# hashicorp/consul

Measured on NVIDIA H100. Metric: million node-ticks/sec, higher is better.
Workload: dtype u32

## Files before the change

### consul_b200/csrc/gs_cuda.cu

```cuda
#include <cuda_runtime.h>
#include <stdio.h>
#include <stdlib.h>
#include <string.h>

#include <map>

#include "gs_aux.h"
#include "gs_backend.h"
#include "gs_query.h"
#include "gs_vmm.h"

#define GS_BLOCK 256
#define GS_GRAPH_TICKS 64
#define GS_WIN_GRAPH 8
#ifndef GS_STRETCH_TICKS
#define GS_STRETCH_TICKS 16
#endif

namespace {

template <bool COORDS>
struct DevSinkT {
  static constexpr bool kCoords = COORDS;
  uint32_t* s_stat;
  uint32_t* s_heard;
  uint32_t* s_q;
  __device__ __forceinline__ void activity() { s_q[0] = 1u; }
  __device__ __forceinline__ void horizon(uint32_t h) { atomicMin(&s_q[1], h); }
  __device__ __forceinline__ void stat(int idx, uint32_t v) { atomicAdd(&s_stat[idx * 32 + (threadIdx.x & 31u)], v); }
  __device__ __forceinline__ void heard(uint32_t r) { atomicAdd(&s_heard[r * 32u + (threadIdx.x & 31u)], 1u); }
  __device__ __forceinline__ void crashed_dead(const GsDev& d, uint32_t t) {
    uint32_t old = atomicSub_system(d.crashed_alive, 1u);
    if (old == 1u) *d.crashed_dead_tick = t;
  }
  __device__ __forceinline__ void log_event(const GsDev& d, const GsGlobals& g, uint32_t t,
                                            uint32_t type, uint32_t subject, uint32_t observer,
                                            uint32_t ltime) {
    uint32_t pos = atomicAdd_system(&d.evlog_cursor[0], 1u);
    if (pos < g.evlog_cap) {
      GsEventRec e;
      e.tick = t;
      e.type = type;
      e.subject = subject;
      e.observer = observer;
      e.ltime = ltime;
      e.reserved = 0u;
      d.evlog[pos] = e;
    } else {
      atomicAdd_system(&d.evlog_cursor[1], 1u);
    }
  }
};
typedef DevSinkT<false> DevSink;

#ifndef GS_MIN_BLOCKS
#define GS_MIN_BLOCKS 4
#endif
#define GS_WARPS (GS_BLOCK / 32)
#define GS_ROUND 4

__device__ __forceinline__ uint32_t gs_smem_addr(const void* p) { return (uint32_t)__cvta_generic_to_shared(p); }
__device__ __forceinline__ void gs_mbar_init(uint64_t* bar, uint32_t arrivals) {
  asm volatile("mbarrier.init.shared::cta.b64 [%0], %1;" ::"r"(gs_smem_addr(bar)), "r"(arrivals) : "memory");
}
__device__ __forceinline__ void gs_mbar_expect_tx(uint64_t* bar, uint32_t bytes) {
  asm volatile("mbarrier.arrive.expect_tx.shared::cta.b64 _, [%0], %1;" ::"r"(gs_smem_addr(bar)), "r"(bytes) : "memory");
}
__device__ __forceinline__ void gs_bulk_g2s(void* smem_dst, const void* gsrc, uint32_t bytes, uint64_t* bar) {
  asm volatile("cp.async.bulk.shared::cluster.global.mbarrier::complete_tx::bytes [%0], [%1], %2, [%3];" ::"r"(
                   gs_smem_addr(smem_dst)),
               "l"(gsrc), "r"(bytes), "r"(gs_smem_addr(bar))
               : "memory");
}
__device__ __forceinline__ bool gs_mbar_wait(uint64_t* bar, uint32_t parity) {
  for (uint32_t spin = 0; spin < (1u << 24); ++spin) {
    uint32_t done;
    asm volatile(
        "{\n\t.reg .pred p;\n\t"
        "mbarrier.try_wait.parity.shared::cta.b64 p, [%1], %2;\n\t"
        "selp.u32 %0, 1, 0, p;\n\t}"
        : "=r"(done)
        : "r"(gs_smem_addr(bar)), "r"(parity)
        : "memory");
    if (done) return true;
  }
  return false;
}

__device__ __forceinline__ void gs_ranks_wait(const GsDev& d, const GsGlobals& g, uint32_t t) {
  if (threadIdx.x < g.world) {
    uint32_t v;
    do {
      asm volatile("ld.acquire.sys.global.u32 %0, [%1];" : "=r"(v) : "l"(d.tick_flags[g.rank] + threadIdx.x) : "memory");
    } while ((int32_t)(v - t) < 0);
  }
  __syncthreads();
}
__device__ __forceinline__ void gs_ranks_release(const GsDev& d, const GsGlobals& g, uint32_t t_done) {
  __syncthreads();
  if (threadIdx.x == 0u) {
    __threadfence_system();
    const uint32_t arrived = atomicAdd(d.done_ctr, 1u);
    if (arrived == gridDim.x - 1u) {
      __threadfence_system();
      *d.done_ctr = 0u;
      __threadfence_system();
      for (uint32_t r = 0; r < g.world; ++r)
        asm volatile("st.release.sys.global.u32 [%0], %1;" ::"l"(d.tick_flags[r] + g.rank), "r"(t_done) : "memory");
    }
  }
}

__device__ __forceinline__ void gs_q_publish(const GsDev& d, const GsGlobals& g, const uint32_t* s_q, uint32_t t) {
  if (s_q[0] != 0u) {
    if (g.world <= 1u) atomicMax(d.qstate[0] + GS_Q_LAST_ACTIVE, t + 1u);
    else for (uint32_t r = 0; r < g.world; ++r) atomicMax_system(d.qstate[r] + GS_Q_LAST_ACTIVE, t + 1u);
  }
  if (s_q[1] != GS_NEVER) {
    if (g.world <= 1u) atomicMin(d.qstate[0] + GS_Q_HORIZON, s_q[1]);
    else for (uint32_t r = 0; r < g.world; ++r) atomicMin_system(d.qstate[r] + GS_Q_HORIZON, s_q[1]);
  }
}

template <bool COORDS>
__device__ __noinline__ void gs_row_step_impaired_call(const GsDev* dp, const GsGlobals* gp, uint32_t i, uint32_t t,
                                                       uint32_t inb, uint32_t* s_stat, uint32_t* s_heard, uint32_t* s_q) {
  DevSinkT<COORDS> sink{s_stat, s_heard, s_q};
  gs_row_step_body<true>(*dp, *gp, i, t, t % gp->GI, inb, sink);
}
template <bool COORDS>
__device__ __noinline__ void gs_row_step_call(const GsDev* dp, const GsGlobals* gp, uint32_t i, uint32_t t,
                                              uint32_t inb, uint32_t* s_stat, uint32_t* s_heard, uint32_t* s_q) {
  if (dp->imp_loss != nullptr) {
    gs_row_step_impaired_call<COORDS>(dp, gp, i, t, inb, s_stat, s_heard, s_q);
    return;
  }
  DevSinkT<COORDS> sink{s_stat, s_heard, s_q};
  gs_row_step_body<false>(*dp, *gp, i, t, t % gp->GI, inb, sink);
}

struct GsStretchCtl {
  GsStretch out;
  uint32_t violation;
  uint32_t end, floor, depth;
};
__device__ __forceinline__ uint32_t gs_stretch_stop(const GsStretchCtl& c, uint32_t last_active) {
  const uint32_t quiet_at = (last_active > c.floor ? last_active : c.floor) + c.depth;
  return quiet_at < c.end ? quiet_at : c.end;
}

template <bool COORDS>
__global__ void __launch_bounds__(GS_BLOCK, GS_MIN_BLOCKS)
    gs_tick_kernel(const __grid_constant__ GsDev d, const GsGlobals* __restrict__ gp, uint32_t k_off,
                   const GsStretchCtl* __restrict__ stretch) {
  __shared__ uint32_t s_stat[GS_NSTAT * 32];
  __shared__ uint32_t s_heard[32 * 32];
  __shared__ __align__(128) uint32_t s_inb[GS_WARPS][GS_ROUND][GS_TILE];
  __shared__ __align__(128) uint32_t s_due[GS_WARPS][GS_ROUND][GS_TILE];
  __shared__ __align__(8) uint64_t s_bar[GS_WARPS];
  __shared__ uint32_t s_q[2];
  __shared__ uint32_t s_work[GS_WARPS * GS_ROUND * 4];
  __shared__ uint32_t s_wn[2], s_wtake[2];
  const uint32_t tid = threadIdx.x;
  for (uint32_t x = tid; x < GS_NSTAT * 32u; x += GS_BLOCK) s_stat[x] = 0u;
  for (uint32_t x = tid; x < 32u * 32u; x += GS_BLOCK) s_heard[x] = 0u;
  if (tid == 64u) s_q[0] = 0u;
  if (tid == 65u) s_q[1] = GS_NEVER;
  if (tid >= 66u && tid < 68u) s_wn[tid - 66u] = 0u;
  if (tid >= 68u && tid < 70u) s_wtake[tid - 68u] = 0u;
  if (tid >= 96u && tid < 96u + GS_WARPS) gs_mbar_init(&s_bar[tid - 96u], 1u);
  asm volatile("fence.mbarrier_init.release.cluster;" ::: "memory");
  asm volatile("griddepcontrol.launch_dependents;" ::: "memory");
  asm volatile("griddepcontrol.wait;" ::: "memory");
  if (stretch != nullptr && *d.tick_base + k_off >= gs_stretch_stop(*stretch, __ldcg(d.qstate[0] + GS_Q_LAST_ACTIVE)))
    return;
  __syncthreads();
  const GsGlobals& g = *gp;
  const uint32_t t = *d.tick_base + k_off;
  if (g.world > 1u) gs_ranks_wait(d, g, t);
  const uint32_t cur = t & 1u, P = g.P, pslot = t % P, gslot = t % g.GI;
  const uint32_t pslot_t = (t + P - g.T % P) % P;
  const uint32_t lane = tid & 31u, wib = tid >> 5;
  uint32_t tile_lo = 0, tile_hi = (g.n + GS_TILE - 1u) / GS_TILE;
  if (g.world > 1u) {
    const uint32_t per = g.rows_per_rank / GS_TILE;
    tile_lo = g.rank * per < tile_hi ? g.rank * per : tile_hi;
    tile_hi = tile_lo + per < tile_hi ? tile_lo + per : tile_hi;
  }
  const uint32_t n_warps = gridDim.x * GS_WARPS, n_tiles = tile_hi - tile_lo;
  const uint32_t wid = blockIdx.x * GS_WARPS + wib;
  const uint32_t t_begin = tile_lo + (uint32_t)(((uint64_t)wid * n_tiles) / n_warps);
  const uint32_t t_end = tile_lo + (uint32_t)(((uint64_t)(wid + 1u) * n_tiles) / n_warps);
  const uint32_t* __restrict__ inbox_cur = d.inbox[t & g.ring_mask];
  const bool gated = g.phase_gate != 0u;
  const uint32_t shift = g.phase_shift;
  DevSinkT<COORDS> sink{s_stat, s_heard, s_q};

  const uint32_t max_run = (n_tiles + n_warps - 1u) / n_warps, n_rounds = (max_run + GS_ROUND - 1u) / GS_ROUND;
  bool did_work = false;
  const bool sys_scan = g.world > 1u && (g.flags & 4u);
  auto bring = [&](uint32_t r) {
    const uint32_t b0 = t_begin + r * GS_ROUND < t_end ? t_begin + r * GS_ROUND : t_end;
    const uint32_t b1 = b0 + GS_ROUND < t_end ? b0 + GS_ROUND : t_end;
    const uint32_t tiles = b1 - b0;
    if (!tiles) return;
    uint32_t gate_mask = 0;
    for (uint32_t x = 0; x < tiles; ++x) {
      bool gate = true;
      if (gated) {
        const uint32_t pp = gs_probe_phase(g.rot_p, (b0 + x) >> shift, P);
        gate = pp == pslot || pp == pslot_t;
      }
      gate_mask |= gate ? 1u << x : 0u;
    }
    const size_t off0 = (size_t)b0 * GS_TILE;
    if (sys_scan) {
      for (uint32_t x = 0; x < tiles; ++x) {
        uint4 v;
        asm volatile("ld.relaxed.sys.global.v4.u32 {%0,%1,%2,%3}, [%4];"
                     : "=r"(v.x), "=r"(v.y), "=r"(v.z), "=r"(v.w) : "l"(inbox_cur + off0 + x * GS_TILE + lane * 4u) : "memory");
        *reinterpret_cast<uint4*>(&s_inb[wib][x][lane * 4u]) = v;
        const uint4 dv = (gate_mask >> x) & 1u ? *reinterpret_cast<const uint4*>(d.due + off0 + x * GS_TILE + lane * 4u)
                                               : make_uint4(GS_NEVER, GS_NEVER, GS_NEVER, GS_NEVER);
        *reinterpret_cast<uint4*>(&s_due[wib][x][lane * 4u]) = dv;
      }
      __syncwarp();
      return;
    }
    for (uint32_t x = 0; x < tiles; ++x)
      if (!((gate_mask >> x) & 1u))
        *reinterpret_cast<uint4*>(&s_due[wib][x][lane * 4u]) = make_uint4(GS_NEVER, GS_NEVER, GS_NEVER, GS_NEVER);
    __syncwarp();
    if (lane == 0u) {
      asm volatile("fence.proxy.async.shared::cta;" ::: "memory");
      gs_mbar_expect_tx(&s_bar[wib], (tiles + __popc(gate_mask)) * GS_TILE * 4u);
      gs_bulk_g2s(&s_inb[wib][0][0], inbox_cur + off0, tiles * GS_TILE * 4u, &s_bar[wib]);
      for (uint32_t x = 0; x < tiles; ++x)
        if ((gate_mask >> x) & 1u) gs_bulk_g2s(&s_due[wib][x][0], d.due + off0 + x * GS_TILE, GS_TILE * 4u, &s_bar[wib]);
    }
  };
  bring(0u);
  for (uint32_t round = 0; round < n_rounds; ++round) {
  const uint32_t par = round & 1u;
  const uint32_t r_begin = t_begin + round * GS_ROUND < t_end ? t_begin + round * GS_ROUND : t_end;
  const uint32_t r_end = r_begin + GS_ROUND < t_end ? r_begin + GS_ROUND : t_end;
  if (r_end > r_begin && !sys_scan && !gs_mbar_wait(&s_bar[wib], round & 1u)) {
    if (lane == 0u) atomicExch(d.qstate[g.rank] + GS_Q_VIOLATION, t + 1u);
  }
  for (uint32_t tile = r_begin; tile < r_end; ++tile) {
    const uint32_t st = tile - r_begin;
    uint4 i4 = *reinterpret_cast<const uint4*>(&s_inb[wib][st][lane * 4u]);
    const uint4 d4 = *reinterpret_cast<const uint4*>(&s_due[wib][st][lane * 4u]);
    if (__any_sync(0xFFFFFFFFu, (i4.x | i4.y | i4.z | i4.w) != 0u)) {
      const uint32_t m0 = tile * GS_TILE + lane * 4u;
      const uint4 h4 = __ldcg(reinterpret_cast<const uint4*>(d.heard + m0));
      uint32_t* const w_cur = d.inbox[t & g.ring_mask] + m0;
      uint32_t* const w4 = &i4.x;
      const uint32_t* const h = &h4.x;
      const uint32_t* const du = &d4.x;
      bool stale_any = false;
#pragma unroll
      for (uint32_t u = 0; u < 4u; ++u) {
        const bool pp = g.pp_interval != 0u && gs_pp_due(g.pp_interval, g.rot_pp, (m0 + u) / g.phase_group, t);
        if (w4[u] != 0u && gs_mail_is_stale(g, w4[u], h[u], du[u] == t, pp)) {
          w_cur[u] = 0u;
          s_inb[wib][st][lane * 4u + u] = 0u;
          w4[u] = 0u;
          stale_any = true;
        }
      }
      if (stale_any) sink.activity();
    }
    bool mine = (i4.x | i4.y | i4.z | i4.w) != 0u || d4.x == t || d4.y == t || d4.z == t || d4.w == t;
    bool pp_tile = false;
    if (g.pp_interval != 0u) {
      if (gated) {
        pp_tile = gs_pp_due(g.pp_interval, g.rot_pp, tile >> shift, t);
      } else {
#pragma unroll
        for (uint32_t u = 0; u < 4u; ++u)
          pp_tile |= gs_pp_due(g.pp_interval, g.rot_pp, (tile * GS_TILE + lane * 4u + u) / g.phase_group, t);
      }
      mine |= pp_tile;
    }
    if (__any_sync(0xFFFFFFFFu, mine)) {
      did_work = true;
      __syncwarp();
      const uint32_t base = tile * GS_TILE + lane;
      bool act[4], cand[4];
      bool any_cand = false;
#pragma unroll
      for (int u = 0; u < 4; ++u) {
        const uint32_t w = s_inb[wib][st][u * 32 + lane];
        const bool due_now = s_due[wib][st][u * 32 + lane] == t;
        act[u] = w != 0u || due_now ||
                 (g.pp_interval != 0u && gs_pp_due(g.pp_interval, g.rot_pp, (base + 32u * u) / g.phase_group, t));
        cand[u] = w == 0u && due_now;
        any_cand |= cand[u];
      }
      if (__any_sync(0xFFFFFFFFu, any_cand)) {
        GsFastProbe f[4];
#pragma unroll
        for (int u = 0; u < 4; ++u)
          if (cand[u]) gs_fast_load(d, cur, base + 32u * u, f[u]);
#pragma unroll
        for (int u = 0; u < 4; ++u)
          if (cand[u]) cand[u] = gs_fast_target(d, g, cur, base + 32u * u, f[u]);
        uint32_t n_probe = 0, n_ack = 0;
#pragma unroll
        for (int u = 0; u < 4; ++u) {
          bool acked = false;
          const bool done = cand[u] && gs_fast_finish(d, g, sink, base + 32u * u, t, f[u], &acked);
          if (done) act[u] = false;
          n_probe += __popc(__ballot_sync(0xFFFFFFFFu, done));
          n_ack += __popc(__ballot_sync(0xFFFFFFFFu, done && acked));
        }
        if (lane == 0u && n_probe) {
          atomicAdd(&s_stat[GS_ST_PROBES * 32], n_probe);
          atomicAdd(&s_stat[GS_ST_ACTIVE_ROWS * 32], n_probe);
          if (n_ack) atomicAdd(&s_stat[GS_ST_ACKS * 32], n_ack);
        }
      }
#pragma unroll
      for (int u = 0; u < 4; ++u) {
        if (__any_sync(0xFFFFFFFFu, act[u]) && lane == 0u) s_work[atomicAdd(&s_wn[par], 1u)] = tile * 4u + (uint32_t)u;
      }
    }
  }
  __syncwarp();
  if (round + 1u < n_rounds) bring(round + 1u);
  __syncthreads();
  if (tid == 0u) s_wn[par ^ 1u] = s_wtake[par ^ 1u] = 0u;
  const uint32_t n_work = s_wn[par];
  for (;;) {
    uint32_t idx = 0;
    if (lane == 0u) idx = atomicAdd(&s_wtake[par], 1u);
    idx = __shfl_sync(0xFFFFFFFFu, idx, 0);
    if (idx >= n_work) break;
    did_work = true;
    const uint32_t i = s_work[idx] * 32u + lane;
    const uint32_t w = __ldcg(inbox_cur + i);
    const bool a = w != 0u || __ldcg(d.due + i) == t ||
                   (g.pp_interval != 0u && gs_pp_due(g.pp_interval, g.rot_pp, i / g.phase_group, t));
    if (a) gs_row_step_call<COORDS>(&d, gp, i, t, w, s_stat, s_heard, s_q);
  }
  __syncthreads();
  }
  if (g.world > 1u && did_work && !(g.flags & 8u)) __threadfence_system();
  __syncthreads();
  if (tid < GS_NSTAT) {
    uint32_t v = 0;
    for (uint32_t x = 0; x < 32u; ++x) v += s_stat[tid * 32u + ((x + tid) & 31u)];
    if (v) atomicAdd(&d.stats[tid], (unsigned long long)v);
  } else if (tid >= 32u && tid < 32u + GS_MAX_RUMORS) {
    uint32_t r = tid - 32u, c = 0;
    for (uint32_t x = 0; x < 32u; ++x) c += s_heard[r * 32u + ((x + r) & 31u)];
    if (c) {
      uint32_t old = atomicAdd_system(&d.heard_cnt[r], c);
      if (old + c == g.up_count) d.conv_tick[r] = t;
    }
  }
  if (tid == 0u) gs_q_publish(d, g, s_q, t);
  if (g.world > 1u) gs_ranks_release(d, g, t + 1u);
}

template <bool COORDS>
__device__ __noinline__ void gs_window_generic(const GsDev* dp, const GsGlobals* gp, uint32_t gb, uint32_t g_end,
                                               uint32_t tf00, uint32_t tf01, uint32_t tf02, uint32_t tf03,
                                               uint32_t tx00, uint32_t tx01, uint32_t tx02, uint32_t tx03,
                                               uint32_t t0, uint32_t w1, uint32_t* s_stat, uint32_t* s_heard,
                                               uint32_t* s_q, uint32_t* counts) {
  const GsDev& d = *dp;
  const GsGlobals& g = *gp;
  const GsHot h = gs_hot(g);
  const uint32_t P = h.P, T = h.T, lane = threadIdx.x & 31u;
  const uint32_t tf0[4] = {tf00, tf01, tf02, tf03}, tx0[4] = {tx00, tx01, tx02, tx03};
  const bool fast_ok =
      h.loss_thr == 0u && h.graph_n == 0u && d.coord == nullptr && d.imp_loss == nullptr && h.pp_interval == 0u;
  DevSinkT<COORDS> sink{s_stat, s_heard, s_q};
  uint32_t n_probe = 0, n_ack = 0;
  bool did_work = false;
  (void)did_work;
#pragma unroll 1
    for (uint32_t s0 = t0; s0 < w1; s0 += P) {
    const uint32_t off = s0 - t0;
    uint32_t tf[4], tx[4], due[4];
    bool cand[4], slow[4];
    bool any_slow = false;
#pragma unroll
    for (int u = 0; u < 4; ++u) {
      if (gb + u < g_end) {
        tf[u] = tf0[u] + off;
        tx[u] = tx0[u] + off;
        due[u] = __ldcg(d.due + (gb + u) * 32u + lane);
      } else {
        tf[u] = tx[u] = GS_NEVER;
        due[u] = GS_NEVER - 1u;
      }
      cand[u] = fast_ok && due[u] == tf[u] && tf[u] < w1;
      slow[u] = (due[u] == tf[u] && tf[u] < w1 && !fast_ok) || (due[u] == tx[u] && tx[u] < w1);
    }
    GsFastProbe f[4];
#pragma unroll
    for (int u = 0; u < 4; ++u)
      if (cand[u]) gs_fast_load(d, tf[u] & 1u, (gb + u) * 32u + lane, f[u]);
#pragma unroll
    for (int u = 0; u < 4; ++u)
      if (cand[u]) {
        const bool okk = gs_fast_target(d, h, tf[u] & 1u, (gb + u) * 32u + lane, f[u]);
        if (!okk) { cand[u] = false; slow[u] = true; }
      }
#pragma unroll
    for (int u = 0; u < 4; ++u) {
      bool acked = false, done = false;
      if (cand[u]) {
        done = gs_fast_finish(d, h, sink, (gb + u) * 32u + lane, tf[u], f[u], &acked);
        if (!done) slow[u] = true;
        else if (!acked && tf[u] + T < w1) slow[u] = true;
      }
      n_probe += done ? 1u : 0u;
      n_ack += done && acked ? 1u : 0u;
      any_slow |= slow[u];
    }
    if (__any_sync(0xFFFFFFFFu, any_slow)) {
      did_work = true;
#pragma unroll 1
      for (int u = 0; u < 4; ++u) {
        const bool sl = u == 0 ? slow[0] : u == 1 ? slow[1] : u == 2 ? slow[2] : slow[3];
        if (!__any_sync(0xFFFFFFFFu, sl)) continue;
        const uint32_t a = u == 0 ? tf[0] : u == 1 ? tf[1] : u == 2 ? tf[2] : tf[3];
        const uint32_t b = u == 0 ? tx[0] : u == 1 ? tx[1] : u == 2 ? tx[2] : tx[3];
        const uint32_t i = (gb + u) * 32u + lane;
#pragma unroll 1
        for (int which = 0; which < 2; ++which) {
          const uint32_t t = which == 0 ? (a < b ? a : b) : (a < b ? b : a);
          if (t >= w1) break;
          if (sl && __ldcg(d.due + i) == t) gs_row_step_call<COORDS>(&d, gp, i, t, 0u, s_stat, s_heard, s_q);
        }
      }
    }
    }
  counts[0] = n_probe;
  counts[1] = n_ack;
}

#ifndef GS_WIN_BLOCKS
#define GS_WIN_BLOCKS 4
#endif
#ifndef GS_WIN_BLOCKS_CLOSED
#define GS_WIN_BLOCKS_CLOSED 4
#endif

template <bool COORDS, bool PRISTINE>
__global__ void __launch_bounds__(GS_BLOCK, PRISTINE ? GS_WIN_BLOCKS_CLOSED : GS_WIN_BLOCKS)
    gs_window_kernel(const __grid_constant__ GsDev d, const GsGlobals* __restrict__ gp, uint32_t k_off, uint32_t n_ticks,
                     uint32_t mode) {
  __shared__ uint32_t s_stat[GS_NSTAT * 32];
  __shared__ uint32_t s_heard[32 * 32];
  __shared__ uint32_t s_q[2];
  __shared__ uint32_t s_spec[GS_MAX_SPECIAL + 1];
  const uint32_t tid = threadIdx.x;
  for (uint32_t x = tid; x < GS_NSTAT * 32u; x += GS_BLOCK) s_stat[x] = 0u;
  for (uint32_t x = tid; x < 32u * 32u; x += GS_BLOCK) s_heard[x] = 0u;
  if (tid == 64u) s_q[0] = 0u;
  if (tid == 65u) s_q[1] = GS_NEVER;
  asm volatile("griddepcontrol.launch_dependents;" ::: "memory");
  asm volatile("griddepcontrol.wait;" ::: "memory");
  if (tid == 66u) s_spec[GS_MAX_SPECIAL] = gs_special_members(*gp, s_spec);
  __syncthreads();
  const GsGlobals& g = *gp;
  const GsHot h = gs_hot(g);
  const bool cyclic = (mode & 2u) != 0u;
  const uint32_t world = g.world, rank = g.rank, n_spec = s_spec[GS_MAX_SPECIAL];
  uint32_t* const qs = d.qstate[rank];
  const uint32_t t0 = *d.tick_base + k_off;
  const uint32_t reached = __ldcg(qs + GS_Q_WIN_END), horizon = __ldcg(qs + GS_Q_HORIZON);
  if (reached < t0) return;
  uint32_t w1 = t0 + n_ticks;
  if (horizon < w1) w1 = horizon;
  if (w1 <= t0) return;
  if (world > 1u) gs_ranks_wait(d, g, t0);
  const uint32_t P = h.P, T = h.T, lane = tid & 31u, wib = tid >> 5;
  uint32_t tile_lo = 0, tile_hi = (h.n + GS_TILE - 1u) / GS_TILE;
  if (world > 1u) {
    const uint32_t per = g.rows_per_rank / GS_TILE;
    tile_lo = rank * per < tile_hi ? rank * per : tile_hi;
    tile_hi = tile_lo + per < tile_hi ? tile_lo + per : tile_hi;
  }
  const uint32_t n_warps = gridDim.x * GS_WARPS, grp_lo = tile_lo * 4u, grp_hi = tile_hi * 4u;
  const uint32_t run = (grp_hi - grp_lo + n_warps - 1u) / n_warps;
  const uint32_t wid = blockIdx.x * GS_WARPS + wib;
  const uint32_t g_begin = grp_lo + wid * run < grp_hi ? grp_lo + wid * run : grp_hi;
  const uint32_t g_end = g_begin + run < grp_hi ? g_begin + run : grp_hi;
  const uint32_t shift = g.phase_shift + 2u, t0_mod = t0 % P, rot_p = g.rot_p;
  const uint32_t win_q = (w1 - t0) / P, win_r = (w1 - t0) - win_q * P;
  const bool fast_ok =
      h.loss_thr == 0u && h.graph_n == 0u && d.coord == nullptr && d.imp_loss == nullptr && h.pp_interval == 0u;
  DevSinkT<COORDS> sink{s_stat, s_heard, s_q};
  bool did_work = false;
  uint32_t n_probe = 0, n_ack = 0;
  uint32_t pg = g_begin >> shift;
  uint32_t pp = (pg % P + rot_p) % P;
  const uint32_t g_first = cyclic ? (grp_lo + wid * 4u < grp_hi ? grp_lo + wid * 4u : grp_hi) : g_begin;
  const uint32_t g_step = cyclic ? n_warps * 4u : 4u, g_lim = cyclic ? grp_hi : g_end;
  for (uint32_t gb = g_first; gb < g_lim; gb += g_step) {
    if (cyclic) {
      pg = gb >> shift;
      pp = (pg % P + rot_p) % P;
    }
    uint32_t tf0[4], tx0[4];
#pragma unroll
    for (int u = 0; u < 4; ++u) {
      const uint32_t grp = gb + u;
      if (grp < g_lim) {
        const uint32_t q = grp >> shift;
        if (q != pg) {
          pp = pp + 1u == P ? 0u : pp + 1u;
          pg = q;
        }
        uint32_t a = pp + P - t0_mod;
        a = a >= P ? a - P : a;
        uint32_t b = a + T;
        b = b >= P ? b - P : b;
        tf0[u] = t0 + a;
        tx0[u] = t0 + b;
      } else {
        tf0[u] = tx0[u] = GS_NEVER;
      }
    }
    uint32_t lo = t0;
#pragma unroll 1
    for (;;) {
      uint32_t stuck = GS_NEVER;
      if constexpr (PRISTINE) {
        uint32_t cnt = 0;
        uint32_t du[4], kk[4], mm[4], cu[4], pa[4];
#pragma unroll
        for (int u = 0; u < 4; ++u) {
          const uint32_t i = (gb + u) * 32u + lane;
          du[u] = GS_NEVER;
          kk[u] = mm[u] = cu[u] = pa[u] = 0u;
          if (gb + u < g_lim) {
            du[u] = __ldcg(d.due + i);
            if (fast_ok) {
              kk[u] = d.key[tf0[u] & 1u][i];
              mm[u] = d.meta[i];
              cu[u] = d.cursor[i];
              pa[u] = d.pass[i];
            }
          }
        }
#pragma unroll
        for (int u = 0; u < 4; ++u) {
          if (gb + u >= g_lim) continue;
          const uint32_t i = (gb + u) * 32u + lane;
          uint32_t due = du[u];
          if (fast_ok && due >= lo && due < w1) {
            uint32_t later = 0u;
            bool on_phase = due == tf0[u];
            if (!on_phase && due > tf0[u]) {
              later = (due - tf0[u]) / P;
              on_phase = later * P == due - tf0[u];
            }
            if (on_phase) {
              const uint32_t k0 = ((due ^ tf0[u]) & 1u) ? d.key[due & 1u][i] : kk[u];
              const uint32_t m = mm[u];
              if (gs_key_truth(k0) == GS_TRUTH_UP && gs_key_rank(k0) == GS_RANK_ALIVE && gs_meta_stage(m) == GS_STAGE_IDLE &&
                  !(m & (GS_META_DIRTY | GS_META_ISOLATED))) {
                const GsU4 rk = gs_perm_keys(h.seed_lo, h.seed_hi, i, pa[u]);
                const uint32_t kt = win_q + (win_r > tf0[u] - t0 ? 1u : 0u) - later;
                const uint32_t k = gs_pristine_probes_k(h.n, h.perm_bits, rk, i, cu[u], kt, s_spec, n_spec);
                if (k) {
                  const uint32_t aw = gs_meta_aw(m);
                  if (aw) d.meta[i] = gs_meta_set_aw(m, aw > k ? aw - k : 0u);
                  d.cursor[i] = cu[u] + k;
                  due += k * P;
                  d.due[i] = due;
                  cnt += k;
                }
              }
            }
          }
          if (due >= lo && due < w1 && due < stuck) stuck = due;
        }
        n_probe += cnt;
        n_ack += cnt;
      } else
      {
        uint32_t mm[4], cu[4], du[4], m_in[4], cu_in[4], du_in[4], kt[4];
        GsU4 rk[4];
        bool live[4], in_rng[4];
        uint32_t cnt = 0;
        {
          uint32_t kk[4], pa[4];
#pragma unroll
          for (int u = 0; u < 4; ++u) {
            const uint32_t i = (gb + u) * 32u + lane;
            in_rng[u] = gb + u < g_lim;
            du[u] = GS_NEVER;
            kk[u] = mm[u] = cu[u] = pa[u] = 0u;
            if (in_rng[u]) {
              du[u] = __ldcg(d.due + i);
              if (fast_ok) {
                kk[u] = d.key[tf0[u] & 1u][i];
                mm[u] = d.meta[i];
                cu[u] = d.cursor[i];
                pa[u] = d.pass[i];
              }
            }
          }
#pragma unroll
          for (int u = 0; u < 4; ++u) {
            const uint32_t i = (gb + u) * 32u + lane;
            live[u] = false;
            kt[u] = 0u;
            m_in[u] = mm[u];
            cu_in[u] = cu[u];
            du_in[u] = du[u];
            if (!in_rng[u] || !fast_ok || du[u] < lo || du[u] >= w1) continue;
            uint32_t later = 0u;
            if (du[u] != tf0[u]) {
              if (du[u] < tf0[u]) continue;
              later = (du[u] - tf0[u]) / P;
              if (later * P != du[u] - tf0[u]) continue;
            }
            const uint32_t k = ((du[u] ^ tf0[u]) & 1u) ? d.key[du[u] & 1u][i] : kk[u];
            live[u] = gs_key_truth(k) == GS_TRUTH_UP && gs_key_rank(k) == GS_RANK_ALIVE &&
                      gs_meta_stage(mm[u]) == GS_STAGE_IDLE && !(mm[u] & (GS_META_DIRTY | GS_META_ISOLATED));
            rk[u] = gs_perm_keys(h.seed_lo, h.seed_hi, i, pa[u]);
            kt[u] = win_q + (win_r > tf0[u] - t0 ? 1u : 0u) - later;
          }
        }
        for (;;) {
          bool go[4];
          bool any = false;
#pragma unroll
          for (int u = 0; u < 4; ++u) {
            go[u] = live[u] && du[u] < w1;
            any |= go[u];
          }
          if (!__any_sync(0xFFFFFFFFu, any)) break;
          uint32_t c[4], kc[4];
#pragma unroll
          for (int u = 0; u < 4; ++u) {
            c[u] = 0u;
            if (go[u]) {
              if (cu[u] >= h.n) {
// ... 1392 lines not shown
```

Baseline: 674,300.

## Compact active rows into per-lane work list instead of per-tile-quarter entries

The work queue changes from one entry per 32-row tile quarter with any active row to one 16-bit entry per active row, packing warp, subtile and lane indices. The drain loop now takes 32 entries per warp at a time, so every lane handles a genuinely active row and the recheck of inbox, due and ping-period conditions is dropped. This is meant to remove warp divergence and idle lanes when active rows are sparse. In exchange it adds ballot/popc compaction and an indirection through s_rtile, and scattered row indices lose coalescing on the inbox load.

```diff
diff --git a/consul_b200/csrc/gs_cuda.cu b/consul_b200/csrc/gs_cuda.cu
--- a/consul_b200/csrc/gs_cuda.cu
+++ b/consul_b200/csrc/gs_cuda.cu
@@ -159,8 +159,10 @@
   __shared__ __align__(128) uint32_t s_due[GS_WARPS][GS_ROUND][GS_TILE];
   __shared__ __align__(8) uint64_t s_bar[GS_WARPS];
   __shared__ uint32_t s_q[2];
-  __shared__ uint32_t s_work[GS_WARPS * GS_ROUND * 4];
+  __shared__ uint16_t s_work[GS_WARPS * GS_ROUND * GS_TILE];
+  __shared__ uint32_t s_rtile[GS_WARPS];
   __shared__ uint32_t s_wn[2], s_wtake[2];
+  static_assert(GS_WARPS <= 8 && GS_ROUND <= 4 && GS_TILE == 128, "s_work entries are 3 + 2 + 7 bits");
   const uint32_t tid = threadIdx.x;
   for (uint32_t x = tid; x < GS_NSTAT * 32u; x += GS_BLOCK) s_stat[x] = 0u;
   for (uint32_t x = tid; x < 32u * 32u; x += GS_BLOCK) s_heard[x] = 0u;
@@ -321,12 +323,26 @@
           if (n_ack) atomicAdd(&s_stat[GS_ST_ACKS * 32], n_ack);
         }
       }
+      uint32_t bal[4], n_act = 0;
 #pragma unroll
       for (int u = 0; u < 4; ++u) {
-        if (__any_sync(0xFFFFFFFFu, act[u]) && lane == 0u) s_work[atomicAdd(&s_wn[par], 1u)] = tile * 4u + (uint32_t)u;
-      }
-    }
-  }
+        bal[u] = __ballot_sync(0xFFFFFFFFu, act[u]);
+        n_act += __popc(bal[u]);
+      }
+      if (n_act) {
+        uint32_t pos = 0;
+        if (lane == 0u) pos = atomicAdd(&s_wn[par], n_act);
+        pos = __shfl_sync(0xFFFFFFFFu, pos, 0);
+        const uint32_t below = (1u << lane) - 1u, key = (wib << 9) | (st << 7) | lane;
+#pragma unroll
+        for (int u = 0; u < 4; ++u) {
+          if (act[u]) s_work[pos + __popc(bal[u] & below)] = (uint16_t)(key | ((uint32_t)u << 5));
+          pos += __popc(bal[u]);
+        }
+      }
+    }
+  }
+  if (lane == 0u) s_rtile[wib] = r_begin;
   __syncwarp();
   if (round + 1u < n_rounds) bring(round + 1u);
   __syncthreads();
@@ -334,15 +350,15 @@
   const uint32_t n_work = s_wn[par];
   for (;;) {
     uint32_t idx = 0;
-    if (lane == 0u) idx = atomicAdd(&s_wtake[par], 1u);
+    if (lane == 0u) idx = atomicAdd(&s_wtake[par], 32u);
     idx = __shfl_sync(0xFFFFFFFFu, idx, 0);
     if (idx >= n_work) break;
     did_work = true;
-    const uint32_t i = s_work[idx] * 32u + lane;
-    const uint32_t w = __ldcg(inbox_cur + i);
-    const bool a = w != 0u || __ldcg(d.due + i) == t ||
-                   (g.pp_interval != 0u && gs_pp_due(g.pp_interval, g.rot_pp, i / g.phase_group, t));
-    if (a) gs_row_step_call<COORDS>(&d, gp, i, t, w, s_stat, s_heard, s_q);
+    if (idx + lane < n_work) {
+      const uint32_t e = s_work[idx + lane];
+      const uint32_t i = (s_rtile[e >> 9] + ((e >> 7) & 3u)) * GS_TILE + (e & 127u);
+      gs_row_step_call<COORDS>(&d, gp, i, t, __ldcg(inbox_cur + i), s_stat, s_heard, s_q);
+    }
   }
   __syncthreads();
   }
```

After: 739,700, median of 6. 9.7% higher.
